# microsoft/UniSpeech

Measured on AMD Instinct MI355X. Metric: audio-seconds/sec pretraining, WavLM-Base 15s@16kHz, higher is better.
Workload: dtype bf16; 1 GPU; WavLM-Base (12L, d=768) pretrain fwd+bwd+grad-reduce+fused-Adam, bf16, batch=32x15s per GPU, masked-pred loss (BASELINE.json configs[1]); global_batch=32, frames_per_utt=749, parallelism=dp1, optimizer=fused Adam, fp32 master, clip 10

## Files before the change

### include/wavlm_hip.h

```cpp
#ifndef WAVLM_HIP_H
#define WAVLM_HIP_H
#include <stddef.h>
#include <stdint.h>
#ifdef __cplusplus
extern "C" {
#endif

#define WAVLM_HIP_ABI_VERSION 30
int wavlm_abi_version(void);

typedef struct wavlm_gemm_desc {
  int32_t dtype;
  int32_t c_dtype;
  int32_t M, N, K, KB;
  int32_t transA, transB;
  int64_t lda, ldb, ldc;
  int64_t sA_kb, sB_kb;
  int32_t batch_o, batch_i;
  int64_t sA_o, sA_i, sB_o, sB_i, sC_o, sC_i;
  const void* A;
  const void* B;
  void* C;
  float alpha;
  int32_t epi;
// ... 188 lines not shown
int wavlm_gumbel_vq_fwd(const void* logits, int32_t dtype, const float* noise, uint64_t seed, float tau, int32_t training,
                        int64_t n, int32_t G, int32_t V, float* ysoft, int32_t* idx, float* part, int64_t ld_part,
                        void* stream);
int wavlm_vq_perplexity(const float* sums, int64_t n, int32_t G, int32_t V, float* out, float* dA, void* stream);
int wavlm_gumbel_vq_bwd(const void* logits, int32_t dtype, const float* ysoft, const float* dret, const float* dA,
                        const float* dppl, float tau, int64_t n, int32_t G, int32_t V, void* dlogits, void* stream);

typedef struct wavlm_layer_desc {
  int32_t B, T, D, H, F;
  int32_t pre_ln;
  int32_t param_dtype;
  int32_t dtab_accumulate;
  float eps1, eps2, scale;
  float p_drop, p_attn;
  int32_t attn_store_p;
  uint64_t seed_r1, seed_r2, seed_attn;
  const void *Wqkv, *bqkv, *Wo, *bo, *W1, *b1, *W2, *b2, *ln1_g, *ln1_b, *ln2_g, *ln2_b;
  const void *Wgate, *bgate, *grep_a;
  void *dWqkv, *dbqkv, *dWo, *dbo, *dW1, *db1, *dW2, *db2, *dln1_g, *dln1_b, *dln2_g, *dln2_b, *dWgate, *dbgate, *dgrep_a;
  void* db2_prev;
  const float* tab;
  const uint8_t* kpm;
  const void* x;
  const void* r_in;
  void* y;
  void* r_out;
  void* saved; uint64_t saved_bytes;
  void* workspace; uint64_t ws_bytes;
  const void* dy;
  const void* dr_out;
  void* dx;
  void* dr_in;
  float* dtab;
} wavlm_layer_desc;
uint64_t wavlm_layer_saved_bytes(const wavlm_layer_desc* d);
uint64_t wavlm_layer_fwd_workspace_bytes(const wavlm_layer_desc* d);
uint64_t wavlm_layer_bwd_workspace_bytes(const wavlm_layer_desc* d);
int wavlm_encoder_layer_fwd(const wavlm_layer_desc* d, void* stream);
int wavlm_encoder_layer_bwd(const wavlm_layer_desc* d, void* stream);

typedef void (*wavlm_grad_listener)(const void* base, uint64_t bytes, void* stream, void* user);
void wavlm_dp_set_listener(wavlm_grad_listener cb, void* user);

int wavlm_dp_unique_id(void* id128);
int wavlm_dp_init(int32_t rank, int32_t world, const void* id128, int32_t average);
int wavlm_dp_bucket_ready(void* base, uint64_t count, int32_t dtype, void* compute_stream);
int wavlm_dp_finish(void* compute_stream);
int wavlm_dp_destroy(void);

uint64_t wavlm_kmeans_centres_bytes(int32_t K, int32_t D);
int wavlm_kmeans_prepare(const float* C, int32_t K, int32_t D, void* image, uint64_t image_bytes, void* stream);
int wavlm_kmeans_assign(const void* X, int32_t x_dtype, int64_t N, int32_t D, int64_t ldx, const void* image, int32_t K,
                        int32_t* labels, float* min_dist, void* stream);
uint64_t wavlm_kmeans_accumulate_workspace_bytes(int64_t N, int32_t K, int32_t D);
int wavlm_kmeans_accumulate(const void* X, int32_t x_dtype, int64_t N, int32_t D, int64_t ldx, const int32_t* labels,
                            int32_t K, float* sums, int32_t* counts, void* workspace, uint64_t ws_bytes, void* stream);
int wavlm_kmeans_update(float* C, float* weights, const float* sums, const int32_t* counts, int32_t K, int32_t D,
                        int32_t mode, void* stream);

int wavlm_spk_mix_norm(const void* const* states, const int64_t* stride_b, const int64_t* stride_t, int32_t n_states,
                       int32_t dtype, const float* weights, const int32_t* lengths, int32_t B, int32_t T, int32_t D,
                       void* out, int32_t out_dtype, int64_t out_stride_b, int64_t out_stride_t, int32_t pad, float add,
                       float eps, void* stream);
int wavlm_spk_rowact(const void* x, int32_t x_dtype, int64_t x_stride_b, int64_t ldx, void* y, int32_t y_dtype,
                     int64_t y_stride_b, int64_t ldy, int32_t B, int32_t T, int32_t C, int32_t act, const float* scale,
                     const float* shift, const int32_t* lengths, float* mean_out, void* stream);
int wavlm_spk_res2(const void* x, int32_t x_dtype, int64_t x_stride_b, int64_t ldx, void* y, int32_t y_dtype,
                   int64_t y_stride_b, int64_t ldy, int32_t B, int32_t T, int32_t C, int32_t dilation, const float* w_image,
                   const float* bias, const float* scale, const float* shift, const int32_t* lengths, void* stream);
uint64_t wavlm_spk_se_workspace_bytes(int32_t B, int32_t C);
int wavlm_spk_se_residual(const void* x, int32_t x_dtype, int64_t x_stride_b, int64_t ldx, const float* mean, const void* w1,
                          const void* b1, const void* w2, const void* b2, int32_t w_dtype, const void* res, int32_t res_dtype,
// ... 110 lines not shown
```

### unispeech_amd/_lib.py

```python
import ctypes as C
import os

_HERE = os.path.dirname(os.path.abspath(__file__))
LIB_PATH = os.environ.get("WAVLM_HIP_LIB") or os.path.join(_HERE, "lib", "libwavlm_hip.so")

_lib = None
ABI_VERSION = 30

F32, BF16, I16 = 0, 1, 2

c_i32, c_i64, c_u64, c_f32, c_vp = C.c_int32, C.c_int64, C.c_uint64, C.c_float, C.c_void_p


class ConvRelayoutDesc(C.Structure):
    _fields_ = [("W", c_vp * 8), ("Wf", c_vp * 8), ("Wb", c_vp * 8),
                ("Cout", c_i32 * 8), ("Cin", c_i32 * 8), ("k", c_i32 * 8), ("s", c_i32 * 8),
                ("n_layers", c_i32), ("dtype", c_i32)]


class GemmDesc(C.Structure):
    _fields_ = [
        ("dtype", c_i32), ("c_dtype", c_i32),
        ("M", c_i32), ("N", c_i32), ("K", c_i32), ("KB", c_i32),
        ("transA", c_i32), ("transB", c_i32),
# ... 4 lines not shown
        ("A", c_vp), ("B", c_vp), ("C", c_vp),
        ("alpha", c_f32), ("epi", c_i32),
        ("bias", c_vp), ("bias_dtype", c_i32), ("sBias_o", c_i64), ("sBias_i", c_i64),
        ("aux", c_vp), ("aux_dtype", c_i32), ("ld_aux", c_i64), ("sAux_o", c_i64), ("sAux_i", c_i64),
        ("res", c_vp), ("res_dtype", c_i32), ("ld_res", c_i64), ("sRes_o", c_i64), ("sRes_i", c_i64),
        ("accumulate", c_i32), ("split_k", c_i32),
        ("workspace", c_vp), ("ws_bytes", c_u64),
        ("colsum", c_vp), ("colsum_dtype", c_i32), ("colsum_accumulate", c_i32),
    ]


class WgradItem(C.Structure):
    _fields_ = [("dy", c_vp), ("x", c_vp), ("dW", c_vp), ("N", c_i32), ("K", c_i32)]


class LayerDesc(C.Structure):
    _fields_ = [
        ("B", c_i32), ("T", c_i32), ("D", c_i32), ("H", c_i32), ("F", c_i32),
        ("pre_ln", c_i32), ("param_dtype", c_i32), ("dtab_accumulate", c_i32),
        ("eps1", c_f32), ("eps2", c_f32), ("scale", c_f32), ("p_drop", c_f32), ("p_attn", c_f32),
        ("attn_store_p", c_i32),
        ("seed_r1", c_u64), ("seed_r2", c_u64), ("seed_attn", c_u64),
        ("Wqkv", c_vp), ("bqkv", c_vp), ("Wo", c_vp), ("bo", c_vp), ("W1", c_vp), ("b1", c_vp), ("W2", c_vp), ("b2", c_vp),
        ("ln1_g", c_vp), ("ln1_b", c_vp), ("ln2_g", c_vp), ("ln2_b", c_vp),
        ("Wgate", c_vp), ("bgate", c_vp), ("grep_a", c_vp),
        ("dWqkv", c_vp), ("dbqkv", c_vp), ("dWo", c_vp), ("dbo", c_vp), ("dW1", c_vp), ("db1", c_vp), ("dW2", c_vp),
        ("db2", c_vp), ("dln1_g", c_vp), ("dln1_b", c_vp), ("dln2_g", c_vp), ("dln2_b", c_vp),
        ("dWgate", c_vp), ("dbgate", c_vp), ("dgrep_a", c_vp),
        ("db2_prev", c_vp),
        ("tab", c_vp), ("kpm", c_vp),
        ("x", c_vp), ("r_in", c_vp), ("y", c_vp), ("r_out", c_vp),
        ("saved", c_vp), ("saved_bytes", c_u64), ("workspace", c_vp), ("ws_bytes", c_u64),
        ("dy", c_vp), ("dr_out", c_vp), ("dx", c_vp), ("dr_in", c_vp), ("dtab", c_vp),
    ]


GRAD_LISTENER = C.CFUNCTYPE(None, c_vp, c_u64, c_vp, c_vp)


SIGNATURES = {
    "wavlm_abi_version": (c_i32, []),
    "wavlm_gemm_workspace_bytes": (c_u64, [C.POINTER(GemmDesc)]),
    "wavlm_gemm": (c_i32, [C.POINTER(GemmDesc), c_vp]),
    "wavlm_gemm_grouped": (c_i32, [C.POINTER(GemmDesc), c_i32, c_vp]),
    "wavlm_grid_blocks": (c_i32, []),
    "wavlm_split_single": (c_i32, [c_i32, c_i32, c_i64, c_i32]),
    "wavlm_split_grouped": (c_i32, [c_i64, c_i64, c_i32, c_i32]),
    "wavlm_slabs_grouped": (c_i32, [c_i64, c_i64, c_i32, c_i32, c_i32]),
    "wavlm_wgrad_grouping": (c_i32, []),
    "wavlm_linear_wgrads_workspace_bytes": (c_u64, [C.POINTER(WgradItem), c_i32, c_i64]),
    "wavlm_linear_wgrads": (c_i32, [C.POINTER(WgradItem), c_i32, c_i64, c_i32, c_vp, c_u64, c_vp]),
    "wavlm_layernorm_fwd": (c_i32, [c_vp, c_vp, c_vp, c_vp, c_vp, c_vp, c_vp, c_vp, c_i64, c_i32, c_f32, c_i32, c_i32,
                                    c_i32, c_f32, c_u64, c_f32, c_u64, c_vp]),
    "wavlm_layernorm_bwd_workspace_bytes": (c_u64, [c_i32]),
    "wavlm_layernorm_bwd": (c_i32, [c_vp, c_vp, c_vp, c_vp, c_vp, c_vp, c_vp, c_vp, c_vp, c_vp, c_vp, c_vp, c_i64, c_i32, c_i32,
                                    c_i32, c_i32, c_f32, c_u64, c_f32, c_u64, c_f32, c_i32, c_i32, c_vp, c_u64, c_vp]),
    "wavlm_layernorm_bwd_seg": (c_i32, [c_vp, c_vp, c_vp, c_vp, c_vp, c_vp, c_vp, c_vp, c_vp, c_vp, c_vp, c_vp, c_i64, c_i32, c_i32,
                                        c_i32, c_i32, c_f32, c_u64, c_f32, c_u64, c_f32, c_i32, c_i32, c_i32, c_i32, c_vp, c_u64,
                                        c_vp]),
    "wavlm_colsum_workspace_bytes": (c_u64, [c_i32]),
    "wavlm_colsum": (c_i32, [c_vp, c_i64, c_i32, c_i64, c_i32, c_vp, c_vp, c_vp, c_i32, c_i32, c_vp, c_u64, c_vp]),
    "wavlm_select_rows": (c_i32, [c_vp, c_vp, c_vp, c_vp, c_vp, c_i64, c_i32, c_i32, c_i32, c_vp]),
    "wavlm_gather_rows": (c_i32, [c_vp, c_vp, c_vp, c_i64, c_i32, c_i32, c_vp]),
    "wavlm_conv_weights_relayout": (c_i32, [C.POINTER(ConvRelayoutDesc), c_vp]),
    "wavlm_conv_wgrad_scatter": (c_i32, [C.POINTER(ConvRelayoutDesc), c_i32, c_vp]),
    "wavlm_axpby": (c_i32, [c_vp, c_i32, c_vp, c_i32, c_i64, c_f32, c_f32, c_vp]),
# ... 47 lines not shown
    "wavlm_posconv_weight_bwd": (c_i32, [c_vp, c_vp, c_vp, c_vp, c_i32, c_vp, c_vp, c_i32, c_i32, c_i32, c_i32, c_vp, c_u64,
                                         c_vp]),
    "wavlm_posconv_direct_supported": (c_i32, [c_i32, c_i32, c_i32]),
    "wavlm_posconv_direct": (c_i32, [c_vp, c_vp, c_vp, c_vp, c_vp, c_vp, c_i32, c_i32, c_i32, c_i32, c_i32, c_i32, c_i32,
                                     c_vp]),
    "wavlm_posconv_group_major": (c_i32, [c_vp, c_vp, c_vp, c_vp, c_i32, c_i32, c_i32, c_i32, c_i32, c_i32, c_i32,
                                          c_i32, c_vp]),
    "wavlm_l2norm_fwd": (c_i32, [c_vp, c_i32, c_vp, c_i32, c_vp, c_i64, c_i32, c_f32, c_vp]),
    "wavlm_l2norm_bwd": (c_i32, [c_vp, c_vp, c_i32, c_vp, c_vp, c_i32, c_i64, c_i32, c_vp]),
    "wavlm_ce_rows": (c_i32, [c_vp, c_vp, c_vp, c_vp, c_vp, c_i32, c_i64, c_i32, c_i64, c_i64, c_f32, c_i32, c_vp]),
    "wavlm_gather_dot": (c_i32, [c_vp, c_vp, c_i32, c_vp, c_vp, c_i64, c_i32, c_i32, c_f32, c_vp, c_vp]),
    "wavlm_rows_wsum": (c_i32, [c_vp, c_i32, c_vp, c_vp, c_vp, c_vp, c_i32, c_i64, c_i32, c_i32, c_vp]),
    "wavlm_bce_workspace_bytes": (c_u64, []),
    "wavlm_bce_logits": (c_i32, [c_vp, c_vp, c_vp, c_vp, c_i64, c_f32, c_vp, c_u64, c_vp]),
    "wavlm_glu_fwd": (c_i32, [c_vp, c_vp, c_i64, c_i32, c_i32, c_i32, c_vp]),
    "wavlm_glu_bwd": (c_i32, [c_vp, c_vp, c_vp, c_i64, c_i32, c_i32, c_i32, c_vp]),
    "wavlm_act_fwd": (c_i32, [c_vp, c_vp, c_i64, c_i32, c_i32, c_vp]),
    "wavlm_act_bwd": (c_i32, [c_vp, c_vp, c_vp, c_i64, c_i32, c_i32, c_vp]),
    "wavlm_sum_workspace_bytes": (c_u64, []),
    "wavlm_sum_f32": (c_i32, [c_vp, c_i64, c_vp, c_vp, c_u64, c_vp]),
    "wavlm_adam_step": (c_i32, [c_vp, c_vp, c_vp, c_vp, c_i32, c_vp, c_i32, c_i64, c_f32, c_f32, c_f32, c_f32, c_f32,
                                c_i64, c_f32, c_vp, c_vp, c_f32, c_vp]),
    "wavlm_mix_workspace_bytes": (c_u64, [c_i32, c_i64]),
    "wavlm_mix_utterances": (c_i32, [c_vp, c_vp, c_vp, c_i32, c_i64, c_vp, c_i32, c_vp, c_vp, c_i32, c_f32, c_vp, c_u64, c_vp]),
    "wavlm_gumbel_vq_partial_rows": (c_u64, [c_i64]),
    "wavlm_gumbel_vq_fwd": (c_i32, [c_vp, c_i32, c_vp, c_u64, c_f32, c_i32, c_i64, c_i32, c_i32, c_vp, c_vp, c_vp, c_i64, c_vp]),
    "wavlm_vq_perplexity": (c_i32, [c_vp, c_i64, c_i32, c_i32, c_vp, c_vp, c_vp]),
    "wavlm_gumbel_vq_bwd": (c_i32, [c_vp, c_i32, c_vp, c_vp, c_vp, c_vp, c_f32, c_i64, c_i32, c_i32, c_vp, c_vp]),
    "wavlm_layer_saved_bytes": (c_u64, [C.POINTER(LayerDesc)]),
    "wavlm_layer_fwd_workspace_bytes": (c_u64, [C.POINTER(LayerDesc)]),
    "wavlm_layer_bwd_workspace_bytes": (c_u64, [C.POINTER(LayerDesc)]),
    "wavlm_encoder_layer_fwd": (c_i32, [C.POINTER(LayerDesc), c_vp]),
    "wavlm_encoder_layer_bwd": (c_i32, [C.POINTER(LayerDesc), c_vp]),
    "wavlm_kmeans_centres_bytes": (c_u64, [c_i32, c_i32]),
    "wavlm_kmeans_prepare": (c_i32, [c_vp, c_i32, c_i32, c_vp, c_u64, c_vp]),
    "wavlm_kmeans_assign": (c_i32, [c_vp, c_i32, c_i64, c_i32, c_i64, c_vp, c_i32, c_vp, c_vp, c_vp]),
    "wavlm_kmeans_accumulate_workspace_bytes": (c_u64, [c_i64, c_i32, c_i32]),
    "wavlm_kmeans_accumulate": (c_i32, [c_vp, c_i32, c_i64, c_i32, c_i64, c_vp, c_i32, c_vp, c_vp, c_vp, c_u64, c_vp]),
    "wavlm_kmeans_update": (c_i32, [c_vp, c_vp, c_vp, c_vp, c_i32, c_i32, c_i32, c_vp]),
    "wavlm_spk_mix_norm": (c_i32, [c_vp, c_vp, c_vp, c_i32, c_i32, c_vp, c_vp, c_i32, c_i32, c_i32, c_vp, c_i32, c_i64, c_i64,
                                   c_i32, c_f32, c_f32, c_vp]),
    "wavlm_spk_rowact": (c_i32, [c_vp, c_i32, c_i64, c_i64, c_vp, c_i32, c_i64, c_i64, c_i32, c_i32, c_i32, c_i32, c_vp, c_vp,
                                 c_vp, c_vp, c_vp]),
    "wavlm_spk_res2": (c_i32, [c_vp, c_i32, c_i64, c_i64, c_vp, c_i32, c_i64, c_i64, c_i32, c_i32, c_i32, c_i32, c_vp, c_vp,
                               c_vp, c_vp, c_vp, c_vp]),
    "wavlm_spk_se_workspace_bytes": (c_u64, [c_i32, c_i32]),
    "wavlm_spk_se_residual": (c_i32, [c_vp, c_i32, c_i64, c_i64, c_vp, c_vp, c_vp, c_vp, c_vp, c_i32, c_vp, c_i32, c_i64, c_i64,
                                      c_vp, c_i32, c_i64, c_i64, c_i32, c_i32, c_i32, c_i32, c_vp, c_vp, c_u64, c_vp]),
    "wavlm_spk_asp": (c_i32, [c_vp, c_i32, c_i64, c_i64, c_vp, c_i32, c_i64, c_i64, c_i32, c_i32, c_i32, c_vp, c_vp, c_vp, c_vp,
                              c_vp, c_i32, c_vp]),
    "wavlm_diar_front": (c_i32, [c_vp, c_vp, c_vp, c_i32, c_i32, c_vp, c_i32, c_i32, c_i32, c_i32, c_i32, c_vp, c_i32, c_i64, c_i64,
                                 c_f32, c_f32, c_vp]),
    "wavlm_attn_plain_fwd": (c_i32, [c_vp, c_vp, c_i32, c_i32, c_i32, c_i32, c_i32, c_f32, c_vp]),
    "wavlm_diar_estimate": (c_i32, [c_vp, c_i32, c_i64, c_i64, c_i32, c_i32, c_i32, c_i32, c_vp, c_vp, c_i32, c_vp]),
    "wavlm_resample_supported": (c_i32, [c_i32, c_i32, c_i32]),
    "wavlm_resample_rows": (c_i32, [c_vp, c_i32, c_i64, c_i32, c_i64, c_vp, c_vp, c_vp, c_i32, c_i32, c_i32, c_vp, c_i32, c_i64,
                                    c_vp]),
    "wavlm_mfcc_supported": (c_i32, [c_i32, c_i32, c_i32]),
    "wavlm_mfcc_frames": (c_i64, [c_i64, c_i32, c_i32]),
    "wavlm_mfcc_rows": (c_i32, [c_vp, c_i32, c_i64, c_i32, c_i64, c_vp, c_i32, c_i32, c_i32, c_vp, c_vp, c_vp, c_vp, c_i32, c_vp,
                                c_vp, c_i64, c_i64, c_i32, c_vp]),
    "wavlm_fbank_supported": (c_i32, [c_i32, c_i32, c_i32, c_i32]),
    "wavlm_fbank_frames": (c_i64, [c_i64, c_i32, c_i32]),
    "wavlm_fbank_rows": (c_i32, [c_vp, c_i32, c_i64, c_i32, c_i64, c_vp, c_i32, c_i32, c_i32, c_i32, c_vp, c_vp, c_vp, c_vp, c_i32,
                                 c_vp, c_i64, c_i64, c_vp]),
    "wavlm_ctc_supported": (c_i32, [c_i32, c_i32]),
# ... 74 lines not shown
```

### unispeech_amd/csrc/attn_fused.hip

```cpp
#include "attn_fused.hpp"

typedef float f32x2_t __attribute__((ext_vector_type(2)));
#if !defined(WAVLM_EXPERIMENTAL)
#undef FA_FWD_LAZY
#undef FA_FWD_THETA
#undef FA_DQ_PK
#endif
#ifndef FA_FWD_LAZY
#define FA_FWD_LAZY 0
#endif
#ifndef FA_FWD_THETA
#define FA_FWD_THETA 8.f
#endif
#ifndef FA_DQ_PK
#define FA_DQ_PK 1
#endif
#if !defined(WAVLM_EXPERIMENTAL)
#undef FA_FWD_MFMA_SUM
#endif
#ifndef FA_FWD_MFMA_SUM
#define FA_FWD_MFMA_SUM 0
#endif
#ifndef FA_FWD_BIAS_IN_C
#define FA_FWD_BIAS_IN_C 1
// ... 999 lines not shown
    if (tab) FA_DQB(true); else FA_DQB(false);
  } else
  if (pstore) {
    if (tab) FA_DQ(false, true, true); else FA_DQ(false, false, true);
  } else if (p.th && p.dbits) {
    if (tab) { if (fa_set_smem(attn_bwd_dq_kernel<true, true, false, false, true>, smem1) != WL_OK) return WL_ELAUNCH;
               WL_LAUNCH((attn_bwd_dq_kernel<true, true, false, false, true>), dim3((unsigned)(nqt * B * H)), dim3(256), smem1, st, p); }
    else { if (fa_set_smem(attn_bwd_dq_kernel<true, false, false, false, true>, smem1) != WL_OK) return WL_ELAUNCH;
           WL_LAUNCH((attn_bwd_dq_kernel<true, false, false, false, true>), dim3((unsigned)(nqt * B * H)), dim3(256), smem1, st, p); }
  } else if (p.th) {
    if (tab) FA_DQ(true, true, false); else FA_DQ(true, false, false);
  } else {
    if (tab) FA_DQ(false, true, false); else FA_DQ(false, false, false);
  }
#undef FA_DQ
#undef FA_DQB
  size_t smem2 = 32768 + (size_t)(p.Ltab + 64) * sizeof(float) + 2 * 4096;
  if (smem2 < FA_CS_FLOATS * sizeof(float)) smem2 = FA_CS_FLOATS * sizeof(float);
  if (use64) {
    p.nqb = (T + FA_K64 - 1) / FA_K64;
    const int rc = fa_launch_dkv64(p, (unsigned)(p.nqb * B * H), st);
    if (rc != WL_OK) return rc;
  } else {
    p.nqb = (T + FA_BK1 - 1) / FA_BK1;
    const dim3 grid2((unsigned)(p.nqb * B * H));
    const int rc = fa_launch_dkv(p, grid2.x, smem2, st);
    if (rc != WL_OK) return rc;
  }
  if (dbias) {
    const int rcb = wl_colsum_finish(p.dbias_part, B * nqt * 4, 3 * H * FA_HD, dbias, dbias_dtype, dbias_accumulate, st);
    if (rcb != WL_OK) return rcb;
    if (dbias_accumulate && !wl_fin_active()) wl_notify_grad(dbias, (uint64_t)3 * H * FA_HD * wl_esize(dbias_dtype), stream);
  }
  if (tab)
    WL_LAUNCH(fa_dtab_reduce_kernel, dim3((unsigned)((Lp / 4 + 15) / 16), (unsigned)H), dim3(1024), 0, st,
              (const float*)p.dtab_part, dtab, (int)B, (int)H, nqt, L, Lp, (int)T, (T + FA_BKV - 1) / FA_BKV, (int)dtab_accumulate);
  return wl_check_launch();
}
```

### unispeech_amd/csrc/common.hpp

```cpp
#pragma once
#include <hip/hip_runtime.h>
#include <stdint.h>
#include <stdio.h>
#include <mutex>

#define WL_MAX_DEVICES 64

#define WL_OK 0
#define WL_EINVAL (-1)
#define WL_ELAUNCH (-2)
#define WL_ENOMEM (-3)

enum { WL_F32 = 0, WL_BF16 = 1, WL_I16 = 2 };

typedef unsigned short bf16_t;

__device__ __forceinline__ float bf2f(bf16_t v) {
  return __uint_as_float(((unsigned)v) << 16);
}
__device__ __forceinline__ bf16_t f2bf(float f) {
  const __bf16 h = (__bf16)f;
  return __builtin_bit_cast(bf16_t, h);
}
__device__ __forceinline__ unsigned pack_bf16x2(float a, float b) {
// ... 146 lines not shown
  } while (0)
int wl_prof_begin(int cls, int dtype, double flops, double bytes, hipStream_t st);
void wl_prof_end(int i, hipStream_t st);
struct WlProfScope {
  int i; hipStream_t st;
  WlProfScope(int cls, int dtype, double flops, double bytes, hipStream_t s) : i(wl_prof_begin(cls, dtype, flops, bytes, s)), st(s) {}
  ~WlProfScope() { wl_prof_end(i, st); }
};

static inline int wl_check_launch() {
  const int e = wl_launch_failed;
  wl_launch_failed = 0;
  return e ? WL_ELAUNCH : WL_OK;
}

void wl_notify_grad(const void* base, uint64_t bytes, void* stream);
static inline uint64_t wl_esize(int dt) { return dt == WL_BF16 ? 2 : 4; }
int wl_attn_fused_bwd_ex(const void* qkv, const void* O, const void* dO, const float* lse, const float* gate,
                         const float* tab, const uint8_t* kpm, const void* pstore, uint64_t pstore_bytes, void* dqkv, float* dgate,
                         float* dtab, int dtab_accumulate,
                         void* dbias, int32_t dbias_dtype, int32_t dbias_accumulate, int32_t B, int32_t H, int32_t T,
                         int32_t head_dim, float scale, float p_drop, uint64_t seed, void* workspace, uint64_t ws_bytes,
                         void* stream);
int wl_colsum_finish(const float* part, int nblk, int n, void* out, int out_dtype, int accumulate, hipStream_t st);

struct WlFinSeg { const float* part; void* out; long stride, rep_stride; int nblk, n, out_dtype, accumulate, rep, blk0; };
#define WL_FIN_MAX 16
struct WlFinList { WlFinSeg s[WL_FIN_MAX]; int n, blocks; };
void wl_fin_defer(WlFinList* l);
bool wl_fin_active();
bool wl_fin_add(const float* part, int nblk, long stride, int n, void* out, int out_dtype, int accumulate, int rep = 1,
                long rep_stride = 0);
int wl_fin_flush(WlFinList& l, void* stream);
```

### unispeech_amd/csrc/layer.hip

```cpp
#include <stdlib.h>
#include <string.h>

#include <atomic>

#include "common.hpp"
#include "split_policy.hpp"
#include "wavlm_hip.h"

static std::atomic<wavlm_grad_listener> g_listener{nullptr};
static std::atomic<void*> g_listener_user{nullptr};
void wl_notify_grad(const void* base, uint64_t bytes, void* stream) {
  const wavlm_grad_listener cb = g_listener.load(std::memory_order_acquire);
  if (cb && base && bytes) cb(base, bytes, stream, g_listener_user.load(std::memory_order_acquire));
}
extern "C" void wavlm_dp_set_listener(wavlm_grad_listener cb, void* user) {
  g_listener.store(nullptr, std::memory_order_release);
  g_listener_user.store(user, std::memory_order_release);
  g_listener.store(cb, std::memory_order_release);
}

namespace {

inline uint64_t rup256(uint64_t v) { return (v + 255) & ~(uint64_t)255; }

struct Carver {
  char* base; uint64_t off, cap; bool ok;
  Carver(void* p, uint64_t bytes) : base((char*)p), off(0), cap(bytes), ok(p != nullptr) {}
  void* take(uint64_t bytes) {
    void* r = base + off;
    off += rup256(bytes);
    if (off > cap) ok = false;
    return r;
  }
};

struct Saved {
// ... 53 lines not shown
int lin_fwd(const void* x, const void* W, const void* b, void* y, int64_t n, int N, int K, int pdt, int epi, void* aux,
            void* stream) {
  wavlm_gemm_desc g; gemm_base(g);
  g.M = (int32_t)n; g.N = N; g.K = K; g.lda = K; g.ldb = K; g.ldc = N;
  g.A = x; g.B = W; g.C = y; g.bias = b; g.bias_dtype = pdt; g.epi = epi;
  if (aux) { g.aux = aux; g.aux_dtype = WL_BF16; g.ld_aux = N; }
  return wavlm_gemm(&g, stream);
}

int lin_dx(const void* dy, const void* W, void* dx, int64_t n, int N, int K, int epi, const void* aux, const void* res,
           void* colsum, int pdt, void* ws, uint64_t wsb, void* stream) {
  wavlm_gemm_desc g; gemm_base(g);
  g.M = (int32_t)n; g.N = K; g.K = N; g.lda = N; g.ldb = K; g.ldc = K; g.transB = 1;
  g.A = dy; g.B = W; g.C = dx; g.epi = epi;
  if (aux) { g.aux = const_cast<void*>(aux); g.aux_dtype = WL_BF16; g.ld_aux = K; }
  if (res) { g.res = res; g.res_dtype = WL_BF16; g.ld_res = K; }
  if (colsum) { g.colsum = colsum; g.colsum_dtype = pdt; g.colsum_accumulate = 1; g.workspace = ws; g.ws_bytes = wsb; }
  return wavlm_gemm(&g, stream);
}
uint64_t lin_dx_colsum_ws(int64_t n, int K) {
  wavlm_gemm_desc g; gemm_base(g);
  g.M = (int32_t)n; g.N = K; g.colsum = (void*)256;
  return wavlm_gemm_workspace_bytes(&g);
}

void wg_desc(wavlm_gemm_desc& g, const wavlm_wgrad_item& w, int64_t n, int pdt, int split) {
  gemm_base(g);
  g.c_dtype = pdt; g.M = w.N; g.N = w.K; g.K = (int32_t)n; g.transA = 1; g.transB = 1;
  g.lda = w.N; g.ldb = w.K; g.ldc = w.K; g.A = w.dy; g.B = w.x; g.C = w.dW; g.accumulate = 1; g.split_k = split;
}
inline long wg_tiles(const wavlm_wgrad_item& w) { return (long)((w.N + 255) / 256) * ((w.K + 255) / 256); }

#define RC(expr) do { const int rc_ = (expr); if (rc_ != WL_OK) return rc_; } while (0)

struct BwdWs {
  void *dsa, *df, *du, *dh, *dxa, *da, *dO, *dqkv;
  float* dgate;
  void *ln_ws, *ln_ws2, *cs_ws, *cs_ws2, *attn_ws, *gate_ws, *wg_ws;
  uint64_t ln_b, cs_b, attn_b, gate_b, wg_b, bytes;
};
BwdWs carve_bwd(const wavlm_layer_desc* d, void* base, uint64_t cap) {
  BwdWs w; memset(&w, 0, sizeof(w));
  Carver c(base ? base : (void*)256, base ? cap : (~(uint64_t)0 >> 1));
  const uint64_t n = (uint64_t)d->B * d->T, D = d->D, F = d->F;
  w.dsa = c.take(n * D * 2);
  w.df = d->p_drop > 0.f ? c.take(n * D * 2) : w.dsa;
  w.du = c.take(n * F * 2);
  w.dh = c.take(n * D * 2);
  w.dxa = c.take(n * D * 2);
  w.da = d->p_drop > 0.f ? c.take(n * D * 2) : w.dxa;
  w.dO = c.take(n * D * 2);
  w.dqkv = c.take(n * 3 * D * 2);
  if (d->tab) w.dgate = (float*)c.take((uint64_t)d->B * d->H * d->T * 4);
  w.ln_b = wavlm_layernorm_bwd_workspace_bytes(d->D); w.ln_ws = c.take(w.ln_b); w.ln_ws2 = c.take(w.ln_b);
  w.cs_b = lin_dx_colsum_ws((int64_t)n, d->F);
  if (w.cs_b < wavlm_colsum_workspace_bytes(d->D)) w.cs_b = wavlm_colsum_workspace_bytes(d->D);
  w.cs_ws = c.take(w.cs_b); w.cs_ws2 = c.take(w.cs_b);
  w.attn_b = wavlm_attn_fused_bwd_workspace_bytes(d->B, d->H, d->T); w.attn_ws = c.take(w.attn_b);
  w.gate_b = wavlm_gate_bwd_workspace_bytes(d->H, 64); w.gate_ws = c.take(w.gate_b);
  const wavlm_wgrad_item it[4] = {{nullptr, nullptr, nullptr, d->D, d->F}, {nullptr, nullptr, nullptr, d->F, d->D},
                                  {nullptr, nullptr, nullptr, d->D, d->D}, {nullptr, nullptr, nullptr, 3 * d->D, d->D}};
  w.wg_b = wavlm_linear_wgrads_workspace_bytes(it, 4, (int64_t)n); w.wg_ws = c.take(w.wg_b);
  w.bytes = c.off;
  if (base && !c.ok) w.bytes = ~(uint64_t)0;
  return w;
}
// ... 148 lines not shown
  WlFinList fin;
  struct Defer { Defer(WlFinList* l) { wl_fin_defer(l); } ~Defer() { wl_fin_defer(nullptr); } } defer(&fin);

  const void* df;
  const void* dres;
  if (!d->pre_ln) {
    RC(wavlm_layernorm_bwd(d->dy, s.s2, s.mean2, s.rstd2, d->ln2_g, d->ln2_b, w.dsa, drop ? w.df : nullptr, nullptr, d->dln2_g,
                           d->dln2_b, d->db2, n, D, WL_BF16, pdt, 0, d->p_drop, d->seed_r2, 0.f, 0, 1.f, 1, 0, w.ln_ws, w.ln_b, stream));
    df = drop ? w.df : w.dsa;
    dres = w.dsa;
  } else {
    df = d->dr_out;
    dres = nullptr;
    if (d->db2)
      RC(wavlm_colsum(df, n, D, D, WL_BF16, nullptr, nullptr, d->db2, pdt, 1, w.cs_ws2, w.cs_b, stream));
  }
  RC(lin_dx(df, d->W2, w.du, n, D, F, 4, s.u, nullptr, d->db1, pdt, w.cs_ws, w.cs_b, stream));
  RC(lin_dx(w.du, d->W1, w.dh, n, F, D, 0, nullptr, dres, nullptr, pdt, nullptr, 0, stream));

  const void* da;
  const void* dxres;
  if (!d->pre_ln) {
    RC(wavlm_layernorm_bwd(w.dh, s.s1, s.mean1, s.rstd1, d->ln1_g, d->ln1_b, w.dxa, drop ? w.da : nullptr, nullptr, d->dln1_g,
                           d->dln1_b, d->dbo, n, D, WL_BF16, pdt, 0, d->p_drop, d->seed_r1, 0.f, 0, 1.f, 1, 0, w.ln_ws2, w.ln_b, stream));
    da = drop ? w.da : w.dxa;
    dxres = w.dxa;
  } else {
    RC(wavlm_layernorm_bwd(w.dh, d->y, s.mean2, s.rstd2, d->ln2_g, d->ln2_b, w.dsa, drop ? w.da : nullptr, d->dy, d->dln2_g,
                           d->dln2_b, d->dbo, n, D, WL_BF16, pdt, 0, d->p_drop, d->seed_r2, 0.f, 0, 1.f, 1, 1, w.ln_ws, w.ln_b, stream));
    da = drop ? w.da : w.dsa;
    dxres = nullptr;
  }
  RC(lin_dx(da, d->Wo, w.dO, n, D, D, 0, nullptr, nullptr, nullptr, pdt, nullptr, 0, stream));
  RC(wl_attn_fused_bwd_ex(s.qkv, s.O, w.dO, s.lse, d->Wgate ? s.gate : nullptr, d->tab, d->kpm, s.pstore, s.pstore_b, w.dqkv, w.dgate, d->dtab,
                          d->dtab_accumulate, d->dbqkv, pdt, 1, d->B, d->H, d->T, 64, d->scale, d->p_attn, d->seed_attn, w.attn_ws,
                          w.attn_b, stream));
  const void* ain = d->pre_ln ? s.h1 : d->x;
  void* dain = d->pre_ln ? w.dxa : d->dx;
  RC(lin_dx(w.dqkv, d->Wqkv, dain, n, 3 * D, D, 0, nullptr, dxres, nullptr, pdt, nullptr, 0, stream));

  const wavlm_wgrad_item it[4] = {{df, s.hact, d->dW2, D, F}, {w.du, s.x1, d->dW1, F, D}, {da, s.O, d->dWo, D, D}, {w.dqkv, ain, d->dWqkv, 3 * D, D}};
  RC(wavlm_linear_wgrads(it, 4, n, pdt, w.wg_ws, w.wg_b, stream));

  if (d->Wgate)
    RC(wavlm_gate_bwd(w.dgate, ain, d->Wgate, d->grep_a, s.ga, s.gb, dain, d->dWgate, d->dbgate, d->dgrep_a, d->B, d->T, d->H, 64,
                      WL_BF16, pdt, 1 | 2, w.gate_ws, w.gate_b, stream));
  if (d->pre_ln) {
    const void* s1 = d->r_in ? s.s1 : d->x;
    RC(wavlm_layernorm_bwd(w.dxa, s1, s.mean1, s.rstd1, d->ln1_g, d->ln1_b, d->dx, (d->r_in && drop) ? d->dr_in : nullptr, w.dsa,
                           d->dln1_g, d->dln1_b, d->r_in ? d->db2_prev : nullptr, n, D, WL_BF16, pdt, 0, d->r_in ? d->p_drop : 0.f,
                           d->seed_r1, 0.f, 0, 1.f, 1, d->r_in ? 1 : 0, w.ln_ws2, w.ln_b, stream));
    if (d->r_in && !drop)
      RC(wavlm_axpby(d->dx, WL_BF16, d->dr_in, WL_BF16, n * D, 1.f, 0.f, stream));
  }
  wl_fin_defer(nullptr);
  return wl_fin_flush(fin, stream);
}

}
```

### unispeech_amd/csrc/rowops.hip

```cpp
#include "common.hpp"
#include <stdlib.h>
#include "../../include/wavlm_hip.h"

__device__ __forceinline__ void load8(const float* p, float (&v)[8]) {
  const float4 a = *reinterpret_cast<const float4*>(p);
  const float4 b = *reinterpret_cast<const float4*>(p + 4);
  v[0] = a.x; v[1] = a.y; v[2] = a.z; v[3] = a.w; v[4] = b.x; v[5] = b.y; v[6] = b.z; v[7] = b.w;
}
__device__ __forceinline__ void load8(const bf16_t* p, float (&v)[8]) {
  const uint4 a = *reinterpret_cast<const uint4*>(p);
  v[0] = __uint_as_float(a.x << 16); v[1] = __uint_as_float(a.x & 0xffff0000u);
  v[2] = __uint_as_float(a.y << 16); v[3] = __uint_as_float(a.y & 0xffff0000u);
  v[4] = __uint_as_float(a.z << 16); v[5] = __uint_as_float(a.z & 0xffff0000u);
  v[6] = __uint_as_float(a.w << 16); v[7] = __uint_as_float(a.w & 0xffff0000u);
}
__device__ __forceinline__ void store8(float* p, const float (&v)[8]) {
  *reinterpret_cast<float4*>(p) = make_float4(v[0], v[1], v[2], v[3]);
  *reinterpret_cast<float4*>(p + 4) = make_float4(v[4], v[5], v[6], v[7]);
}
__device__ __forceinline__ void store8(bf16_t* p, const float (&v)[8]) {
  uint4 o;
  o.x = pack_bf16x2(v[0], v[1]); o.y = pack_bf16x2(v[2], v[3]);
  o.z = pack_bf16x2(v[4], v[5]); o.w = pack_bf16x2(v[6], v[7]);
  *reinterpret_cast<uint4*>(p) = o;
// ... 554 lines not shown
    for (; b < nblk; b += 64) s0 += part[(long)b * stride + c];
    s = (s0 + s1) + (s2 + s3);
  }
  red[slice][col] = s;
  __syncthreads();
  if (slice < 4) {
    float t = 0.f;
#pragma unroll
    for (int k = 0; k < 16; ++k) t += red[slice * 16 + k][col];
    red[slice * 16][col] = t;
  }
  __syncthreads();
  if (slice == 0 && c < n) {
    s = (red[0][col] + red[16][col]) + (red[32][col] + red[48][col]);
    for (int r = 0; r < g.rep; ++r) {
      const long idx = (long)r * g.rep_stride + c;
      st_elem(g.out, idx, g.out_dtype, g.accumulate ? s + ld_elem(g.out, idx, g.out_dtype) : s);
    }
  }
}

static thread_local WlFinList* g_fin_list = nullptr;
void wl_fin_defer(WlFinList* l) { g_fin_list = l; if (l) { l->n = 0; l->blocks = 0; } }
bool wl_fin_active() { return g_fin_list != nullptr; }
bool wl_fin_add(const float* part, int nblk, long stride, int n, void* out, int out_dtype, int accumulate, int rep, long rep_stride) {
  WlFinList* l = g_fin_list;
  if (!l || l->n >= WL_FIN_MAX || n <= 0) return false;
  WlFinSeg& g = l->s[l->n++];
  g.part = part; g.out = out; g.stride = stride; g.rep_stride = rep_stride; g.nblk = nblk; g.n = n; g.out_dtype = out_dtype;
  g.accumulate = accumulate; g.rep = rep < 1 ? 1 : rep; g.blk0 = l->blocks;
  l->blocks += (n + 15) / 16;
  return true;
}
int wl_fin_flush(WlFinList& l, void* stream) {
  if (l.n == 0) return WL_OK;
  WL_LAUNCH(colsum_finish_multi_kernel, dim3((unsigned)l.blocks), dim3(1024), 0, (hipStream_t)stream, l);
  const int rc = wl_check_launch();
  if (rc == WL_OK)
    for (int k = 0; k < l.n; ++k) {
      const WlFinSeg& g = l.s[k];
      if (g.accumulate) wl_notify_grad(g.out, (uint64_t)((long)(g.rep - 1) * g.rep_stride + g.n) * wl_esize(g.out_dtype), stream);
    }
  l.n = 0; l.blocks = 0;
  return rc;
}

#define CS_MAXC 8
template <typename T>
__global__ __launch_bounds__(256) void colsum_partial_kernel(const T* __restrict__ x, long rows, int N, long ld,
    const unsigned char* __restrict__ inc, const unsigned char* __restrict__ exc, float* __restrict__ part) {
  __shared__ float red[4][512];
  const int lane = threadIdx.x & 63, wave = threadIdx.x >> 6;
  const int nch = N >> 3;
  float acc[CS_MAXC][8];
#pragma unroll
  for (int c = 0; c < CS_MAXC; ++c)
#pragma unroll
    for (int e = 0; e < 8; ++e) acc[c][e] = 0.f;
  for (long row = (long)blockIdx.x * 4 + wave; row < rows; row += (long)gridDim.x * 4) {
    if (inc && !inc[row]) continue;
    if (exc && exc[row]) continue;
#pragma unroll
    for (int c = 0; c < CS_MAXC; ++c) {
      const int ch = lane + 64 * c;
      if (ch < nch) {
        float v[8];
        load8(x + row * ld + ch * 8, v);
#pragma unroll
        for (int e = 0; e < 8; ++e) acc[c][e] += v[e];
      }
    }
  }
  float* pg = part + (long)blockIdx.x * N;
#pragma unroll
  for (int c = 0; c < CS_MAXC; ++c) {
// ... 595 lines not shown
```

### unispeech_amd/functional.py

```python
import os
import threading
import weakref

import torch

from . import ops

_SEED_CTR = [0]
USE_FUSED_ATTENTION = True
_ASP = os.environ.get("WAVLM_ATTN_STORE_P", "0")
ATTN_STORE_P = True if _ASP == "1" else ("bits" if _ASP in ("bits", "2") else False)


def next_seed():
    _SEED_CTR[0] += 1
    return (torch.initial_seed() * 0x9E3779B97F4A7C15 + _SEED_CTR[0] * 0xD1B54A32D192ED03) & 0xFFFFFFFFFFFFFFFF


def _rup(x, m):
    return (x + m - 1) // m * m


CHAIN_CONSUMERS = os.environ.get("WAVLM_CHAIN_CONSUMERS", "1") == "1"
WGRAD_GROUPING = None
SINK_LISTENERS = []


def h2d(a, dev):
    t = torch.from_numpy(a) if not torch.is_tensor(a) else a
    dev = torch.device(dev)
    if dev.type != "cuda" or t.device.type != "cpu" or t.numel() == 0:
        return t.to(dev)
    return t.pin_memory().to(dev, non_blocking=True)


_SINK_USES = {}


def reset_sink_uses():
    _SINK_USES.clear()
    _PADDED_GRAD[0] = None


def _sink_use(p, explicit=None):
# ... 1085 lines not shown
```

### unispeech_amd/layerfn.py

```python
import ctypes as C
import os
import weakref

import torch

from . import _lib, ops
from . import functional as F

LAYER_FUSED = os.environ.get("WAVLM_LAYER_FUSED", "1") != "0"


class TabGrad:
    __slots__ = ("buf",)

    def __init__(self):
        self.buf = None


def _ptr(t):
    return t.data_ptr() if t is not None else None


class _Binding:

# ... 151 lines not shown
        if d.pre_ln:
            if dy is None or dr_out is None:
                raise NotImplementedError("fused pre-LN block: both outputs must be used")
            dr_out = dr_out if dr_out.is_contiguous() else dr_out.contiguous()
            d.dr_out = dr_out.data_ptr()
            d.y = y.data_ptr()
        dy = dy if dy.is_contiguous() else dy.contiguous()
        d.dy = dy.data_ptr()
        dx = torch.empty_like(xc)
        d.dx = dx.data_ptr()
        dr_in = None
        if rc is not None:
            dr_in = torch.empty_like(xc)
            d.dr_in = dr_in.data_ptr()
        tg = ctx.tabgrad
        if ctx.use_tab:
            d.dWgate, d.dbgate, d.dgrep_a = bd.gate_grad_ptrs
            if tg.buf is None:
                tg.buf = torch.empty_like(tab)
                d.dtab_accumulate = 0
            else:
                d.dtab_accumulate = 1
            d.dtab = tg.buf.data_ptr()
        b2_here = True
        if d.pre_ln:
            b2_here = not (ctx.out_tok is not None and ctx.out_tok.taken)
            if not b2_here:
                d.db2 = None
            d.db2_prev = _ptr(ctx.prev_sink)
        L = _lib.lib()
        need = int(L.wavlm_layer_bwd_workspace_bytes(C.byref(d)))
        ws = ops.workspace(dev, need, "layer")
        d.workspace, d.ws_bytes = ws.data_ptr(), need
        _lib.check(L.wavlm_encoder_layer_bwd(C.byref(d), ops.stream()), "wavlm_encoder_layer_bwd")
        if F.SINK_LISTENERS:
            for i, (_p, g) in enumerate(bd.sinks):
                if i == bd.b2_index and not b2_here:
                    continue
                F._sink_written(g)
            if ctx.use_tab:
                for g in bd.gate_sinks:
                    F._sink_written(g)
            if ctx.prev_sink is not None:
                F._sink_written(ctx.prev_sink)
        dtab = tg.buf if (ctx.use_tab and ctx.owns_tab) else None
        return dx, dr_in, dtab, None, None, None, None, None, None


def run_block(layer, x, kpm, table, r_in=None, prev_tok=None, out_tok=None):
    at = layer.self_attn
    if at.has_relative_attention_bias and table is None:
        table = at.position_table(x.shape[1], x.device)
    tab_in, tg, owns = None, None, False
    if table is not None:
        tg = getattr(table, "_wl_tabgrad", None)
        if tg is None:
            tg = table._wl_tabgrad = TabGrad()
            owns = True
        tab_in = table if owns else table.detach()
    out = EncoderLayerFn.apply(x, r_in, tab_in, layer, kpm, tg, owns, prev_tok, out_tok)
    if layer.layer_norm_first:
        return out[0], out[1], table
    return out, None, table
```

### unispeech_amd/ops.py

```python
import ctypes as C
import math
import os

import torch

from . import _lib
from ._lib import BF16, F32, ConvRelayoutDesc, GemmDesc, check

_WS = {}


def dt(t):
    if t.dtype == torch.float32:
        return F32
    if t.dtype == torch.bfloat16:
        return BF16
    raise TypeError("unsupported dtype %s (float32 / bfloat16 only)" % t.dtype)


def _dev(t):
    if not t.is_cuda:
        raise _lib.WavlmHipError("unispeech_amd kernels need a HIP device tensor (no CPU fallback)")
    return t.device


_RAW_STREAM = getattr(torch._C, "_cuda_getCurrentRawStream", None)


def stream():
    if _RAW_STREAM is not None:
        return C.c_void_p(_RAW_STREAM(torch.cuda.current_device()))
    return C.c_void_p(torch.cuda.current_stream().cuda_stream)


def ptr(t, offset=0):
    if t is None:
        return None
    return C.c_void_p(t.data_ptr() + offset * t.element_size())


WS_MIN_BYTES = 10 << 20


def workspace(device, nbytes, tag="main"):
    key = (device.index, tag, _RAW_STREAM(device.index) if _RAW_STREAM is not None else torch.cuda.current_stream(device).cuda_stream)
    buf = _WS.get(key)
    if buf is None or buf.numel() < nbytes:
        buf = torch.empty(max(int(nbytes), WS_MIN_BYTES), dtype=torch.uint8, device=device)
        _WS[key] = buf
    return buf


def _contig(t):
    if t is not None and not t.is_contiguous():
        raise ValueError("expected a contiguous tensor")
    return t


def gemm(A, B, Cc, M, N, K, *, lda, ldb, ldc, transA=False, transB=False, KB=1, sA_kb=0, sB_kb=0, batch=(1, 1),
         sA=(0, 0), sB=(0, 0), sC=(0, 0), a_off=0, b_off=0, c_off=0, alpha=1.0, bias=None, bias_off=0, sBias=(0, 0),
         epi=0, aux=None, aux_off=0, ld_aux=0, sAux=(0, 0), res=None, res_off=0, ld_res=0, sRes=(0, 0),
         accumulate=False, split_k=1, colsum=None, colsum_accumulate=False):
    dev = _dev(A)
    if A.dtype != B.dtype:
        raise TypeError("A and B must share a dtype")
    d = GemmDesc()
    d.dtype, d.c_dtype = dt(A), dt(Cc)
    d.M, d.N, d.K, d.KB = int(M), int(N), int(K), int(KB)
    d.transA, d.transB = int(bool(transA)), int(bool(transB))
    d.lda, d.ldb, d.ldc = int(lda), int(ldb), int(ldc)
    d.sA_kb, d.sB_kb = int(sA_kb), int(sB_kb)
    d.batch_o, d.batch_i = int(batch[0]), int(batch[1])
    d.sA_o, d.sA_i = int(sA[0]), int(sA[1])
    d.sB_o, d.sB_i = int(sB[0]), int(sB[1])
    d.sC_o, d.sC_i = int(sC[0]), int(sC[1])
    d.A, d.B, d.C = ptr(A, a_off), ptr(B, b_off), ptr(Cc, c_off)
    d.alpha, d.epi = float(alpha), int(epi)
    d.bias = ptr(bias, bias_off)
    d.bias_dtype = dt(bias) if bias is not None else 0
    d.sBias_o, d.sBias_i = int(sBias[0]), int(sBias[1])
    d.aux = ptr(aux, aux_off)
    d.aux_dtype = dt(aux) if aux is not None else 0
    d.ld_aux, d.sAux_o, d.sAux_i = int(ld_aux), int(sAux[0]), int(sAux[1])
# ... 1087 lines not shown
```

Baseline: 15430 audio-s/s.

## Overlap gate backward and dtab reduce on an auxiliary stream during layer backward

```diff
diff --git a/include/wavlm_hip.h b/include/wavlm_hip.h
--- a/include/wavlm_hip.h
+++ b/include/wavlm_hip.h
@@ -244,12 +244,15 @@
   void* dx;
   void* dr_in;
   float* dtab;
+  void* aux;
 } wavlm_layer_desc;
 uint64_t wavlm_layer_saved_bytes(const wavlm_layer_desc* d);
 uint64_t wavlm_layer_fwd_workspace_bytes(const wavlm_layer_desc* d);
 uint64_t wavlm_layer_bwd_workspace_bytes(const wavlm_layer_desc* d);
 int wavlm_encoder_layer_fwd(const wavlm_layer_desc* d, void* stream);
 int wavlm_encoder_layer_bwd(const wavlm_layer_desc* d, void* stream);
+int wavlm_aux_create(void** ctx);
+int wavlm_aux_destroy(void* ctx);
 
 typedef void (*wavlm_grad_listener)(const void* base, uint64_t bytes, void* stream, void* user);
 void wavlm_dp_set_listener(wavlm_grad_listener cb, void* user);
diff --git a/unispeech_amd/_lib.py b/unispeech_amd/_lib.py
--- a/unispeech_amd/_lib.py
+++ b/unispeech_amd/_lib.py
@@ -60,6 +60,7 @@
         ("x", c_vp), ("r_in", c_vp), ("y", c_vp), ("r_out", c_vp),
         ("saved", c_vp), ("saved_bytes", c_u64), ("workspace", c_vp), ("ws_bytes", c_u64),
         ("dy", c_vp), ("dr_out", c_vp), ("dx", c_vp), ("dr_in", c_vp), ("dtab", c_vp),
+        ("aux", c_vp),
     ]
 
 
@@ -173,6 +174,8 @@
     "wavlm_layer_bwd_workspace_bytes": (c_u64, [C.POINTER(LayerDesc)]),
     "wavlm_encoder_layer_fwd": (c_i32, [C.POINTER(LayerDesc), c_vp]),
     "wavlm_encoder_layer_bwd": (c_i32, [C.POINTER(LayerDesc), c_vp]),
+    "wavlm_aux_create": (c_i32, [C.POINTER(c_vp)]),
+    "wavlm_aux_destroy": (c_i32, [c_vp]),
     "wavlm_kmeans_centres_bytes": (c_u64, [c_i32, c_i32]),
     "wavlm_kmeans_prepare": (c_i32, [c_vp, c_i32, c_i32, c_vp, c_u64, c_vp]),
     "wavlm_kmeans_assign": (c_i32, [c_vp, c_i32, c_i64, c_i32, c_i64, c_vp, c_i32, c_vp, c_vp, c_vp]),
diff --git a/unispeech_amd/csrc/attn_fused.hip b/unispeech_amd/csrc/attn_fused.hip
--- a/unispeech_amd/csrc/attn_fused.hip
+++ b/unispeech_amd/csrc/attn_fused.hip
@@ -1055,8 +1055,16 @@
     if (rcb != WL_OK) return rcb;
     if (dbias_accumulate && !wl_fin_active()) wl_notify_grad(dbias, (uint64_t)3 * H * FA_HD * wl_esize(dbias_dtype), stream);
   }
-  if (tab)
+  if (tab && dtab_accumulate != WL_DTAB_DEFER)
     WL_LAUNCH(fa_dtab_reduce_kernel, dim3((unsigned)((Lp / 4 + 15) / 16), (unsigned)H), dim3(1024), 0, st,
               (const float*)p.dtab_part, dtab, (int)B, (int)H, nqt, L, Lp, (int)T, (T + FA_BKV - 1) / FA_BKV, (int)dtab_accumulate);
   return wl_check_launch();
 }
+
+int wl_attn_fused_dtab_reduce(const void* workspace, float* dtab, int dtab_accumulate, int32_t B, int32_t H, int32_t T, void* stream) {
+  if (!workspace || !dtab || B <= 0 || H <= 0 || T <= 0) return WL_EINVAL;
+  const int nqt = (T + FA_BQ - 1) / FA_BQ, L = 2 * T - 1, Lp = (L + 3) & ~3;
+  WL_LAUNCH(fa_dtab_reduce_kernel, dim3((unsigned)((Lp / 4 + 15) / 16), (unsigned)H), dim3(1024), 0, (hipStream_t)stream,
+            (const float*)workspace, dtab, (int)B, (int)H, nqt, L, Lp, (int)T, (T + FA_BKV - 1) / FA_BKV, (int)(dtab_accumulate != 0));
+  return wl_check_launch();
+}
diff --git a/unispeech_amd/csrc/common.hpp b/unispeech_amd/csrc/common.hpp
--- a/unispeech_amd/csrc/common.hpp
+++ b/unispeech_amd/csrc/common.hpp
@@ -202,3 +202,13 @@
 bool wl_fin_add(const float* part, int nblk, long stride, int n, void* out, int out_dtype, int accumulate, int rep = 1,
                 long rep_stride = 0);
 int wl_fin_flush(WlFinList& l, void* stream);
+int wl_fin_launch(const WlFinList& l, void* stream);
+void wl_fin_notify(WlFinList& l, void* stream);
+
+struct WlAux {
+  hipStream_t st;
+  hipEvent_t fork, join;
+  std::mutex mu;
+};
+#define WL_DTAB_DEFER 2
+int wl_attn_fused_dtab_reduce(const void* workspace, float* dtab, int dtab_accumulate, int32_t B, int32_t H, int32_t T, void* stream);
diff --git a/unispeech_amd/csrc/layer.hip b/unispeech_amd/csrc/layer.hip
--- a/unispeech_amd/csrc/layer.hip
+++ b/unispeech_amd/csrc/layer.hip
@@ -2,6 +2,7 @@
 #include <string.h>
 
 #include <atomic>
+#include <new>
 
 #include "common.hpp"
 #include "split_policy.hpp"
@@ -121,6 +122,31 @@
 inline long wg_tiles(const wavlm_wgrad_item& w) { return (long)((w.N + 255) / 256) * ((w.K + 255) / 256); }
 
 #define RC(expr) do { const int rc_ = (expr); if (rc_ != WL_OK) return rc_; } while (0)
+#define HC(expr) do { if ((expr) != hipSuccess) return WL_ELAUNCH; } while (0)
+
+struct AuxLock {
+  WlAux* a;
+  explicit AuxLock(WlAux* x) : a(x) { if (a) a->mu.lock(); }
+  ~AuxLock() { if (a) a->mu.unlock(); }
+};
+struct AuxFork {
+  WlAux* a; hipEvent_t ev; hipStream_t main; bool open;
+  AuxFork() : a(nullptr), ev(nullptr), main(nullptr), open(false) {}
+  int begin(WlAux* x, hipEvent_t fork, hipEvent_t join_ev, void* stream) {
+    a = x; ev = join_ev; main = (hipStream_t)stream;
+    HC(hipStreamWaitEvent(a->st, fork, 0));
+    open = true;
+    return WL_OK;
+  }
+  int join() {
+    if (!open) return WL_OK;
+    open = false;
+    HC(hipEventRecord(ev, a->st));
+    HC(hipStreamWaitEvent(main, ev, 0));
+    return WL_OK;
+  }
+  ~AuxFork() { (void)join(); }
+};
 
 struct BwdWs {
   void *dsa, *df, *du, *dh, *dxa, *da, *dO, *dqkv;
@@ -335,19 +361,35 @@
     dxres = nullptr;
   }
   RC(lin_dx(da, d->Wo, w.dO, n, D, D, 0, nullptr, nullptr, nullptr, pdt, nullptr, 0, stream));
+  WlAux* const aux = (d->Wgate && !g_listener.load(std::memory_order_acquire)) ? (WlAux*)d->aux : nullptr;
+  AuxLock lock(aux);
+  AuxFork fork;
   RC(wl_attn_fused_bwd_ex(s.qkv, s.O, w.dO, s.lse, d->Wgate ? s.gate : nullptr, d->tab, d->kpm, s.pstore, s.pstore_b, w.dqkv, w.dgate, d->dtab,
-                          d->dtab_accumulate, d->dbqkv, pdt, 1, d->B, d->H, d->T, 64, d->scale, d->p_attn, d->seed_attn, w.attn_ws,
-                          w.attn_b, stream));
+                          aux ? WL_DTAB_DEFER : (d->dtab_accumulate != 0), d->dbqkv, pdt, 1, d->B, d->H, d->T, 64, d->scale, d->p_attn,
+                          d->seed_attn, w.attn_ws, w.attn_b, stream));
   const void* ain = d->pre_ln ? s.h1 : d->x;
   void* dain = d->pre_ln ? w.dxa : d->dx;
   RC(lin_dx(w.dqkv, d->Wqkv, dain, n, 3 * D, D, 0, nullptr, dxres, nullptr, pdt, nullptr, 0, stream));
+  if (aux) HC(hipEventRecord(aux->fork, (hipStream_t)stream));
 
   const wavlm_wgrad_item it[4] = {{df, s.hact, d->dW2, D, F}, {w.du, s.x1, d->dW1, F, D}, {da, s.O, d->dWo, D, D}, {w.dqkv, ain, d->dWqkv, 3 * D, D}};
   RC(wavlm_linear_wgrads(it, 4, n, pdt, w.wg_ws, w.wg_b, stream));
 
-  if (d->Wgate)
+  bool fin_launched = false;
+  if (aux) {
+    RC(fork.begin(aux, aux->fork, aux->join, stream));
+    RC(wavlm_gate_bwd(w.dgate, ain, d->Wgate, d->grep_a, s.ga, s.gb, dain, d->dWgate, d->dbgate, d->dgrep_a, d->B, d->T, d->H, 64,
+                      WL_BF16, pdt, 1 | 2, w.gate_ws, w.gate_b, aux->st));
+    RC(wl_attn_fused_dtab_reduce(w.attn_ws, d->dtab, d->dtab_accumulate, d->B, d->H, d->T, aux->st));
+    if (!d->pre_ln) {
+      RC(wl_fin_launch(fin, aux->st));
+      fin_launched = true;
+    }
+    RC(fork.join());
+  } else if (d->Wgate) {
     RC(wavlm_gate_bwd(w.dgate, ain, d->Wgate, d->grep_a, s.ga, s.gb, dain, d->dWgate, d->dbgate, d->dgrep_a, d->B, d->T, d->H, 64,
                       WL_BF16, pdt, 1 | 2, w.gate_ws, w.gate_b, stream));
+  }
   if (d->pre_ln) {
     const void* s1 = d->r_in ? s.s1 : d->x;
     RC(wavlm_layernorm_bwd(w.dxa, s1, s.mean1, s.rstd1, d->ln1_g, d->ln1_b, d->dx, (d->r_in && drop) ? d->dr_in : nullptr, w.dsa,
@@ -357,7 +399,36 @@
       RC(wavlm_axpby(d->dx, WL_BF16, d->dr_in, WL_BF16, n * D, 1.f, 0.f, stream));
   }
   wl_fin_defer(nullptr);
+  if (fin_launched) {
+    wl_fin_notify(fin, stream);
+    return WL_OK;
+  }
   return wl_fin_flush(fin, stream);
 }
 
-}
+int wavlm_aux_create(void** ctx) {
+  if (!ctx) return WL_EINVAL;
+  *ctx = nullptr;
+  WlAux* a = new (std::nothrow) WlAux();
+  if (!a) return WL_ENOMEM;
+  a->st = nullptr;
+  hipEvent_t* ev[2] = {&a->fork, &a->join};
+  for (hipEvent_t* e : ev) *e = nullptr;
+  bool ok = hipStreamCreateWithFlags(&a->st, hipStreamNonBlocking) == hipSuccess;
+  for (hipEvent_t* e : ev) ok = ok && hipEventCreateWithFlags(e, hipEventDisableTiming) == hipSuccess;
+  if (!ok) { wavlm_aux_destroy(a); return WL_ELAUNCH; }
+  *ctx = a;
+  return WL_OK;
+}
+
+int wavlm_aux_destroy(void* ctx) {
+  if (!ctx) return WL_OK;
+  WlAux* a = (WlAux*)ctx;
+  hipEvent_t ev[2] = {a->fork, a->join};
+  for (hipEvent_t e : ev) if (e) (void)hipEventDestroy(e);
+  if (a->st) (void)hipStreamDestroy(a->st);
+  delete a;
+  return WL_OK;
+}
+
+}
diff --git a/unispeech_amd/csrc/rowops.hip b/unispeech_amd/csrc/rowops.hip
--- a/unispeech_amd/csrc/rowops.hip
+++ b/unispeech_amd/csrc/rowops.hip
@@ -610,15 +610,21 @@
   l->blocks += (n + 15) / 16;
   return true;
 }
-int wl_fin_flush(WlFinList& l, void* stream) {
+int wl_fin_launch(const WlFinList& l, void* stream) {
   if (l.n == 0) return WL_OK;
   WL_LAUNCH(colsum_finish_multi_kernel, dim3((unsigned)l.blocks), dim3(1024), 0, (hipStream_t)stream, l);
-  const int rc = wl_check_launch();
-  if (rc == WL_OK)
-    for (int k = 0; k < l.n; ++k) {
-      const WlFinSeg& g = l.s[k];
-      if (g.accumulate) wl_notify_grad(g.out, (uint64_t)((long)(g.rep - 1) * g.rep_stride + g.n) * wl_esize(g.out_dtype), stream);
-    }
+  return wl_check_launch();
+}
+void wl_fin_notify(WlFinList& l, void* stream) {
+  for (int k = 0; k < l.n; ++k) {
+    const WlFinSeg& g = l.s[k];
+    if (g.accumulate) wl_notify_grad(g.out, (uint64_t)((long)(g.rep - 1) * g.rep_stride + g.n) * wl_esize(g.out_dtype), stream);
+  }
+  l.n = 0; l.blocks = 0;
+}
+int wl_fin_flush(WlFinList& l, void* stream) {
+  const int rc = wl_fin_launch(l, stream);
+  if (rc == WL_OK) wl_fin_notify(l, stream);
   l.n = 0; l.blocks = 0;
   return rc;
 }
diff --git a/unispeech_amd/functional.py b/unispeech_amd/functional.py
--- a/unispeech_amd/functional.py
+++ b/unispeech_amd/functional.py
@@ -10,6 +10,7 @@
 USE_FUSED_ATTENTION = True
 _ASP = os.environ.get("WAVLM_ATTN_STORE_P", "0")
 ATTN_STORE_P = True if _ASP == "1" else ("bits" if _ASP in ("bits", "2") else False)
+AUX_STREAM = os.environ.get("WAVLM_AUX_STREAM", "1") != "0"
 
 
 def next_seed():
diff --git a/unispeech_amd/layerfn.py b/unispeech_amd/layerfn.py
--- a/unispeech_amd/layerfn.py
+++ b/unispeech_amd/layerfn.py
@@ -207,6 +207,7 @@
         need = int(L.wavlm_layer_bwd_workspace_bytes(C.byref(d)))
         ws = ops.workspace(dev, need, "layer")
         d.workspace, d.ws_bytes = ws.data_ptr(), need
+        d.aux = ops.aux_context(dev) if (F.AUX_STREAM and not F.SINK_LISTENERS) else None
         _lib.check(L.wavlm_encoder_layer_bwd(C.byref(d), ops.stream()), "wavlm_encoder_layer_bwd")
         if F.SINK_LISTENERS:
             for i, (_p, g) in enumerate(bd.sinks):
diff --git a/unispeech_amd/ops.py b/unispeech_amd/ops.py
--- a/unispeech_amd/ops.py
+++ b/unispeech_amd/ops.py
@@ -1,3 +1,4 @@
+import atexit
 import ctypes as C
 import math
 import os
@@ -49,6 +50,28 @@
         buf = torch.empty(max(int(nbytes), WS_MIN_BYTES), dtype=torch.uint8, device=device)
         _WS[key] = buf
     return buf
+
+
+_AUX = {}
+
+
+def aux_context(device):
+    idx = device.index if device.index is not None else torch.cuda.current_device()
+    ctx = _AUX.get(idx)
+    if ctx is None:
+        h = C.c_void_p()
+        with torch.cuda.device(idx):
+            check(_lib.lib().wavlm_aux_create(C.byref(h)), "wavlm_aux_create")
+        if not _AUX:
+            atexit.register(_aux_destroy_all)
+        ctx = _AUX[idx] = h.value
+    return ctx
+
+
+def _aux_destroy_all():
+    while _AUX:
+        _, ctx = _AUX.popitem()
+        _lib.lib().wavlm_aux_destroy(C.c_void_p(ctx))
 
 
 def _contig(t):
```

After: 14350 audio-s/s. 7.0% lower.
